# mauro3/KissMCMC.jl

Measured on AMD Instinct MI355X. Metric: walker-steps/sec, higher is better.
Workload: dtype f64

## Files before the change

### include/kissmcmc_hip.h

```cpp
#ifndef KISSMCMC_HIP_H
#define KISSMCMC_HIP_H

#include <stdint.h>

#ifdef __cplusplus
extern "C" {
#endif

#define KMC_VERSION 100

typedef enum kmc_status {
    KMC_OK = 0,
    KMC_ERR_A_SCALE = 1,
    KMC_ERR_ODD_WALKERS = 2,
    KMC_ERR_TOO_FEW_WALKERS = 3,
    KMC_ERR_BAD_ARG = 4,
    KMC_ERR_NONFINITE_LOGP = 5,
    KMC_ERR_HIP = 6,
    KMC_ERR_OOM = 7,
    KMC_ERR_NO_DEVICE = 8,
    KMC_ERR_UNSUPPORTED = 9
} kmc_status;

typedef enum kmc_density {
// ... 403 lines not shown
                                      int64_t* tail_len_j, int64_t* n_reff_nan, int64_t* n_out, int64_t* info);
kmc_status  kmc_chain_psis_loo_reff(kmc_user_density* density, const double* params, const double* chain_host, int64_t nsamples, int64_t nwalkers,
                                    int64_t ndim, int64_t first_sample, const uint8_t* walker_mask, int64_t thin, const double* r_eff_j,
                                    int32_t split, int64_t max_lag, int64_t obs_first, int64_t obs_count, int64_t workspace_bytes, int device,
                                    double* stats, double* lppd_j, double* r_eff_used, int64_t* tail_len_j, int64_t* n_reff_nan, int64_t* n_out,
                                    int64_t* info);
kmc_status  kmc_sampler_psis_tail_reff(kmc_sampler* s, int64_t first_sample, const uint8_t* walker_mask, int64_t thin, const double* r_eff_j,
                                       int32_t split, int64_t max_lag, int64_t obs_first, int64_t obs_count, int64_t workspace_bytes, double* tail,
                                       double* m_j, double* xc_j, int32_t* n_tail_j, int64_t* tail_len, double* r_eff_used, int64_t* tail_len_j,
                                       int64_t* n_reff_nan, int64_t* n_out);
kmc_status  kmc_chain_psis_tail_reff(kmc_user_density* density, const double* params, const double* chain_host, int64_t nsamples, int64_t nwalkers,
                                     int64_t ndim, int64_t first_sample, const uint8_t* walker_mask, int64_t thin, const double* r_eff_j,
                                     int32_t split, int64_t max_lag, int64_t obs_first, int64_t obs_count, int64_t workspace_bytes, int device,
                                     double* tail, double* m_j, double* xc_j, int32_t* n_tail_j, int64_t* tail_len, double* r_eff_used,
                                     int64_t* tail_len_j, int64_t* n_reff_nan, int64_t* n_out);

kmc_status  kmc_debug_accept_terms(uint64_t seed, uint64_t step, uint64_t walker0, int64_t n, int64_t nhalf, double a_scale,
                                   int64_t ndim, int device, int64_t* partner_host, double* z_host, double* t1_host, double* lu_host);
kmc_status  kmc_debug_chain_by_walker(const void* src_host, int is_float, int64_t K, int64_t nl, int64_t ld, int64_t nd, int64_t w0,
                                      int64_t nw, int64_t dst_stride, double* dst_host, int64_t dst_len, int device);
kmc_status  kmc_debug_rows_compact(const double* src_host, int64_t rows, int64_t ld, int64_t nd, double* dst_host, int64_t dst_len,
                                   int device);
int         kmc_debug_phase_spec(int density, int L, int K, int iter);

#ifdef __cplusplus
}
#endif
#endif
```

### kissmcmc.jl_amd/_lib.py

```python
from __future__ import annotations

import ctypes as C
import os

_HERE = os.path.dirname(os.path.abspath(__file__))
LIB_PATH = os.environ.get("KMC_LIB_PATH") or os.path.join(_HERE, "libkissmcmc_hip.so")

OK, ERR_A_SCALE, ERR_ODD_WALKERS, ERR_TOO_FEW_WALKERS, ERR_BAD_ARG, ERR_NONFINITE_LOGP, \
    ERR_HIP, ERR_OOM, ERR_NO_DEVICE, ERR_UNSUPPORTED = range(10)
GAUSSIAN_ISO, EXPONENTIAL, ROSENBROCK, LOGNORMAL, MVNORMAL2 = range(5)
USER_DENSITY = 100
HOST_DENSITY = 101
DATA_DENSITY = 102
HOST_LOGPDF_FN = C.CFUNCTYPE(C.c_int, C.POINTER(C.c_double), C.c_int64, C.c_int64, C.POINTER(C.c_double), C.c_void_p)
HOST_PROPOSE_FN = C.CFUNCTYPE(C.c_int, C.POINTER(C.c_double), C.c_int64, C.c_int64, C.POINTER(C.c_double), C.c_void_p)
HOST_ACCEPTED_FN = C.CFUNCTYPE(C.c_int, C.POINTER(C.c_uint8), C.c_int64, C.c_int64, C.c_int64, C.c_int32, C.c_void_p)
F64 = 0
F32 = 1
STORE_CHAIN, STORE_LOGP, MOMENTS, NO_GRAPH, P2P, ISLANDS, P2P_FINEGRAINED, P2P_PUSH = 1, 2, 4, 8, 16, 64, 128, 512
STREAM_CHAIN = 2048
CHAIN_BY_WALKER = 4096
STORE_BLOBS = 8192
MOVE_STRETCH, MOVE_DE, MOVE_SNOOKER, MOVE_MIX = 0, 1, 3, 4
MIX_MAX = 4
TEMPS_MAX = 64
CONV_NEED_LAGS, CONV_TRUNCATED = 1, 2
CONV_HAS_NAN = 4
TEMPER_WHOLE, TEMPER_LIKELIHOOD = 0, 1
P2P_HANDLE_BYTES = 128
RCCL_ID_BYTES = 128

SYMBOLS = [
    "kmc_version", "kmc_device_count", "kmc_last_error", "kmc_status_string", "kmc_validate",
    "kmc_g_pdf", "kmc_cdf_g_inv", "kmc_emcee_run", "kmc_sampler_create", "kmc_sampler_destroy",
    "kmc_sampler_set_stream", "kmc_sampler_bind_positions", "kmc_sampler_p2p_export", "kmc_sampler_p2p_connect", "kmc_sampler_p2p_connect_local", "kmc_sampler_p2p_link_probe", "kmc_sampler_set_positions", "kmc_sampler_init_ball", "kmc_sampler_set_state", "kmc_sampler_run", "kmc_sampler_half_step",
    "kmc_sampler_sync", "kmc_sampler_last_run_ms", "kmc_sampler_generation", "kmc_sampler_nsamples",
    "kmc_sampler_launch_count", "kmc_sampler_describe", "kmc_sampler_device_ptr", "kmc_sampler_get_positions",
    "kmc_sampler_get_logp", "kmc_sampler_get_naccept", "kmc_sampler_get_accept_ratio",
    "kmc_sampler_get_moments", "kmc_sampler_get_chain", "kmc_sampler_get_chain_by_walker", "kmc_logpdf_eval", "kmc_logpdf_eval_host",
    "kmc_user_density_create", "kmc_user_density_create_body", "kmc_user_density_destroy", "kmc_metropolis_validate", "kmc_metropolis_run", "kmc_cholesky_lower", "kmc_int_acorr", "kmc_sampler_int_acorr",
    "kmc_sizeof_config", "kmc_sizeof_metropolis_config", "kmc_sizeof_outputs", "kmc_sizeof_metropolis_outputs", "kmc_deal_seed", "kmc_deal_perm", "kmc_sampler_deal_pack", "kmc_sampler_deal_unpack",
    "kmc_sampler_get_walker_ids", "kmc_sampler_set_walker_ids", "kmc_sampler_set_chain_host", "kmc_rccl_unique_id", "kmc_sampler_rccl_init",
    "kmc_sampler_rccl_capture", "kmc_sampler_rccl_set_capture", "kmc_rccl_version", "kmc_device_free_bytes",
    "kmc_sampler_launch_mode", "kmc_updated_budget", "kmc_set_updated_budget_mb", "kmc_debug_accept_terms",
    "kmc_debug_chain_by_walker", "kmc_debug_rows_compact", "kmc_debug_phase_spec",
    "kmc_user_density_create_body_blob", "kmc_user_density_nblob", "kmc_logpdf_blob_eval_host", "kmc_sampler_get_blobs",
    "kmc_device_cache_release", "kmc_user_density_is_separable", "kmc_host_prefault", "kmc_data_density_create",
    "kmc_sampler_get_rung_state", "kmc_sampler_set_rung_state", "kmc_sampler_get_swaps",
    "kmc_sampler_get_rung_loglike", "kmc_sampler_set_rung_loglike_sum", "kmc_sampler_get_ladder", "kmc_sampler_set_ladder",
    "kmc_sampler_order_stats", "kmc_sampler_chain_argmax", "kmc_chain_order_stats", "kmc_chain_argmax",
    "kmc_sampler_histograms", "kmc_chain_histograms", "kmc_hist_pair_plan",
    "kmc_sampler_lag_sums", "kmc_chain_lag_sums", "kmc_convergence_stats", "kmc_sampler_convergence", "kmc_chain_convergence",
    "kmc_convergence_plan",
    "kmc_rank_plan", "kmc_rank_normal_scores", "kmc_sampler_rank_scores", "kmc_chain_rank_scores", "kmc_sampler_rank_convergence",
    "kmc_chain_rank_convergence",
    "kmc_sampler_hdi", "kmc_chain_hdi", "kmc_hdi_span",
    "kmc_sampler_covariance", "kmc_chain_covariance", "kmc_cov_plan", "kmc_cov_correlation",
    "kmc_sampler_pointwise_stats", "kmc_chain_pointwise_stats", "kmc_sampler_pointwise_loglike", "kmc_chain_pointwise_loglike",
    "kmc_pointwise_plan", "kmc_waic_stats",
    "kmc_sampler_psis_loo", "kmc_chain_psis_loo", "kmc_sampler_psis_tail", "kmc_chain_psis_tail", "kmc_psis_plan", "kmc_loo_stats",
    "kmc_psis_smooth_host",
    "kmc_sampler_relative_eff", "kmc_chain_relative_eff", "kmc_sampler_pointwise_weights", "kmc_chain_pointwise_weights",
    "kmc_sampler_psis_loo_reff", "kmc_chain_psis_loo_reff", "kmc_sampler_psis_tail_reff", "kmc_chain_psis_tail_reff",
]


class Config(C.Structure):
    _fields_ = [
# ... 265 lines not shown
    L.kmc_sampler_set_walker_ids.argtypes = [vp, ip]
    L.kmc_sampler_set_chain_host.argtypes = [vp, dp, dp]
    L.kmc_rccl_unique_id.argtypes = [vp]
    L.kmc_sampler_rccl_init.argtypes = [vp, vp]
    L.kmc_sampler_rccl_capture.argtypes = [vp, C.POINTER(C.c_int)]
    L.kmc_sampler_rccl_set_capture.argtypes = [vp, C.c_int]
    L.kmc_rccl_version.argtypes = [C.POINTER(C.c_int), C.c_char_p, C.c_int64]
    L.kmc_device_free_bytes.argtypes = [C.c_int, C.POINTER(C.c_uint64), C.POINTER(C.c_uint64)]
    L.kmc_device_cache_release.argtypes = []
    L.kmc_device_cache_release.restype = None
    L.kmc_host_prefault.argtypes = [C.c_void_p, C.c_uint64, C.c_int]
    L.kmc_host_prefault.restype = None
    L.kmc_sampler_launch_mode.restype = C.c_int
    L.kmc_sampler_launch_mode.argtypes = [vp, C.POINTER(C.c_int)]
    L.kmc_updated_budget.restype = None
    L.kmc_updated_budget.argtypes = [ip, ip]
    L.kmc_set_updated_budget_mb.restype = None
    L.kmc_set_updated_budget_mb.argtypes = [C.c_double]
    L.kmc_debug_accept_terms.argtypes = [C.c_uint64, C.c_uint64, C.c_uint64, C.c_int64, C.c_int64, C.c_double, C.c_int64, C.c_int, ip, dp, dp, dp]
    L.kmc_debug_chain_by_walker.argtypes = [vp, C.c_int, C.c_int64, C.c_int64, C.c_int64, C.c_int64, C.c_int64, C.c_int64, C.c_int64, dp, C.c_int64, C.c_int]
    L.kmc_debug_rows_compact.argtypes = [dp, C.c_int64, C.c_int64, C.c_int64, dp, C.c_int64, C.c_int]
    L.kmc_debug_phase_spec.restype = C.c_int
    L.kmc_debug_phase_spec.argtypes = [C.c_int, C.c_int, C.c_int, C.c_int]
    for fn, T in ((L.kmc_sizeof_config, Config), (L.kmc_sizeof_metropolis_config, MetropolisConfig),
                  (L.kmc_sizeof_outputs, Outputs), (L.kmc_sizeof_metropolis_outputs, MetropolisOutputs)):
        if fn() != C.sizeof(T):
            raise ImportError(f"{LIB_PATH}: struct layout mismatch ({fn.__name__}() = {fn()}, the ctypes mirror {T.__name__} is {C.sizeof(T)} bytes): "
                              "rebuild the library or update kissmcmc_jl_amd/_lib.py from include/kissmcmc_hip.h")
    _lib = L
    return L


def check(status: int) -> None:
    if status != OK:
        L = lib()
        msg = L.kmc_last_error().decode() or L.kmc_status_string(status).decode()
        raise KmcError(status, msg)
```

### kissmcmc.jl_amd/build.py

```python
from __future__ import annotations

import os
import shutil
import subprocess

_HERE = os.path.dirname(os.path.abspath(__file__))
CSRC = os.path.join(_HERE, "csrc")
LIB = os.path.join(_HERE, "libkissmcmc_hip.so")
SOURCES = ["kmc_sampler.hip", "kmc_plan.hip", "kmc_launch.hip", "kmc_updated.hip", "kmc_state.hip", "kmc_copy.hip", "kmc_rtc.hip", "kmc_p2p.hip", "kmc_metropolis_api.hip", "kmc_acorr.hip", "kmc_summary.hip", "kmc_hist.hip", "kmc_convergence.hip", "kmc_rank.hip", "kmc_hdi.hip", "kmc_cov.hip", "kmc_pointwise.hip", "kmc_rccl.hip", "kmc_diag.hip", "kmc_inst_host.hip", "kmc_inst_host_temper.hip", "kmc_inst_host_temper_snooker.hip", "kmc_data.hip"] + \
          [f"kmc_inst_{d}{part}.hip" for part in ("", "_var", "_p2p", "_lds", "_spec", "_de", "_snooker", "_temper", "_temper_snooker") for d in ("lognormal", "exponential", "gaussian_iso", "rosenbrock", "mvnormal2")]
HEADERS = ["kmc_psis_fit.hpp", "kmc_host.hpp", "kmc_sampler.hpp", "kmc_device.hpp", "kmc_kernels.hpp", "kmc_islands.hpp", "kmc_generation.hpp", "kmc_copy_kernels.hpp", "kmc_summary_kernels.hpp", "kmc_hist_kernels.hpp", "kmc_convergence_kernels.hpp", "kmc_convergence_host.hpp", "kmc_rank_kernels.hpp", "kmc_rank_host.hpp", "kmc_hdi_kernels.hpp", "kmc_cov_kernels.hpp", "kmc_chain_view.hpp", "kmc_chain_kernels.hpp", "kmc_metropolis.hpp", "kmc_tables.hpp", "kmc_recognise.hpp", "kmc_data.hpp", "kmc_pointwise.hpp", os.path.join("..", "..", "include", "kissmcmc_hip.h")]
PRELOAD = ["-mllvm", "-amdgpu-kernarg-preload-count=14"]
FLAGS = ["--offload-arch=gfx950", "-O3", "-std=c++17", "-fPIC", "-ffp-contract=off",
         "-fvisibility=hidden", "-Wall", "-Wno-unused-function"]


def _hipcc() -> str:
    for c in (shutil.which("hipcc"), "/opt/rocm/bin/hipcc"):
        if c and os.path.exists(c):
            return c
    raise RuntimeError("hipcc not found: the HIP library cannot be built")




def stale(lib: str = LIB) -> bool:
    if not os.path.exists(lib):
        return True
    t = os.path.getmtime(lib)
    deps = [os.path.join(CSRC, f) for f in SOURCES + HEADERS]
    return any(os.path.getmtime(d) > t for d in deps)


def build(force: bool = False, verbose: bool = False, extra_flags=(), out: str = LIB, preload: bool = True) -> str:
# ... 30 lines not shown
```

### kissmcmc.jl_amd/csrc/kmc_plan.hip

```cpp
#include <algorithm>
#include <cmath>
#include <cstdlib>
#include <cstring>

#include "kmc_sampler.hpp"

using namespace kmc;
using namespace kmc_host;

namespace kmc_host {
bool lookup(int density, int L, int K, int iter, bool p2p, bool ragged, bool f32, HalfStepFn* vec, HalfStepFn* gen)
{
    return with_density(density, false, [&](auto d) {
        using D = decltype(d);
        if (p2p && f32) { *vec = nullptr; *gen = nullptr; }
        else if (p2p) density_part<D, 2>(L, K, iter, ragged, false, vec, gen);
        else if (ragged || f32) density_part<D, 1>(L, K, iter, ragged, f32, vec, gen);
        else density_part<D, 0>(L, K, iter, false, false, vec, gen);
        return true;
    });
}

bool lookup_move(int move, int density, int L, int K, int iter, bool ragged, HalfStepFn* vec, HalfStepFn* gen)
{
    return with_density(density, false, [&](auto d) {
        if (move == KMC_MOVE_SNOOKER) density_part<decltype(d), 4>(L, K, iter, ragged, false, vec, gen);
        else if (move == KMC_MOVE_MIX) density_part<decltype(d), 5>(L, K, iter, ragged, false, vec, gen);
        else density_part<decltype(d), 3>(L, K, iter, ragged, false, vec, gen);
        return true;
    });
}

bool lookup_temper(int move, int density, int L, int K, int iter, bool ragged, HalfStepFn* vec, HalfStepFn* gen)
{
    return with_density(density, false, [&](auto d) {
        using D = decltype(d);
        if (move == KMC_MOVE_SNOOKER) temper_part<D, Move::Snooker>(L, K, iter, ragged, vec, gen);
        else if (move == KMC_MOVE_MIX) temper_part<D, Move::Mix>(L, K, iter, ragged, vec, gen);
        else if (move == KMC_MOVE_DE) temper_part<D, Move::DE>(L, K, iter, ragged, vec, gen);
        else temper_part<D, Move::Stretch>(L, K, iter, ragged, vec, gen);
        return true;
    });
}

HalfStepFn lookup_spec(int density, int L, int K, int iter)
{
    return with_density(density, HalfStepFn(nullptr), [&](auto d) { return spec_part<decltype(d)>(L, K, iter); });
}

LogpdfFn logpdf_fn(int density)
{
    return with_density(density, LogpdfFn(nullptr), [](auto d) { return logpdf_lookup<decltype(d)>(); });
}

bool resident_lane_wanted(int64_t ndim)
{
    std::string e;
    if (debug_opt("resident", &e) && e == "pair") return false;
    return ndim <= 8;
}
int lane_nd(int64_t ndim) { return (int)ndim; }

void philox_host(const uint32_t ctr[4], const uint32_t key[2], uint32_t out[4])
{
    uint32_t c0 = ctr[0], c1 = ctr[1], c2 = ctr[2], c3 = ctr[3], k0 = key[0], k1 = key[1];
    for (int r = 0; r < 10; ++r) {
        const uint64_t p0 = (uint64_t)0xD2511F53u * c0, p1 = (uint64_t)0xCD9E8D57u * c2;
        const uint32_t n0 = (uint32_t)(p1 >> 32) ^ c1 ^ k0, n2 = (uint32_t)(p0 >> 32) ^ c3 ^ k1;
        c0 = n0; c1 = (uint32_t)p1; c2 = n2; c3 = (uint32_t)p0;
        k0 += 0x9E3779B9u; k1 += 0xBB67AE85u;
// ... 72 lines not shown
            if (c.move == KMC_MOVE_SNOOKER) temper_part<HostEval, Move::Snooker>(1, 1, 1, false, &vec, &p.fn);
            else if (c.move == KMC_MOVE_MIX) temper_part<HostEval, Move::Mix>(1, 1, 1, false, &vec, &p.fn);
            else if (c.move == KMC_MOVE_DE) temper_part<HostEval, Move::DE>(1, 1, 1, false, &vec, &p.fn);
            else temper_part<HostEval, Move::Stretch>(1, 1, 1, false, &vec, &p.fn);
        }
        return p;
    }
    if (c.density == KMC_USER_DENSITY) {
        const kmc_user_density* ud = static_cast<const kmc_user_density*>(c.user_density);
        const bool body = ud && ud->is_body && !(sep_routed(ud) || body_vec_possible(ud, c.ndim));
        if (!body && !force_generic && L > 0 && 2 * L * K >= c.ndim && iter <= L && iter * K <= 16) {
            if (ud && ud->is_body && !sep_routed(ud)) while (iter > 1 && body_vec_lds_bytes(L, K, iter) > 65536) iter /= 2;
            p.vec = true; p.L = L; p.K = K; p.ITER = iter;
        } else {
            p.vec = false; p.L = 1; p.K = 1; p.ITER = 1;
        }
        return p;
    }
    if (tempered(c)) lookup_temper(c.move, c.density, L, K, iter, ragged, &vec, &gen);
    else if (de) lookup_move(c.move, c.density, L, K, iter, ragged, &vec, &gen);
    else lookup(c.density, L, K, iter, (c.flags & KMC_P2P) != 0, ragged, f32, &vec, &gen);
    if (!force_generic && L > 0 && 2 * L * K >= c.ndim && vec != nullptr) {
        p.fn = vec; p.vec = true; p.L = L; p.K = K; p.ITER = iter;
        if (!tempered(c) && !de && !(c.flags & KMC_P2P) && !ragged && !f32 && iter <= 2) p.fn_credit = lookup_spec(c.density, L, K, iter);
    } else {
        p.fn = gen; p.vec = false; p.L = 1; p.K = 1; p.ITER = 1;
    }
    return p;
}

kmc_status check_ndim(int density, int64_t ndim)
{
    if (density == KMC_ROSENBROCK && ndim < 2) return fail(KMC_ERR_BAD_ARG, "rosenbrock needs ndim >= 2");
    if (density == KMC_MVNORMAL2 && ndim != 2) return fail(KMC_ERR_BAD_ARG, "mvnormal2 needs ndim == 2");
    return KMC_OK;
}

}
kmc_status kmc_host::digest_params(const kmc_config& c, DensityParams* dp)
{
    for (double& v : dp->p) v = 0.0;
    dp->ndim = (int32_t)c.ndim;
    dp->pad_ = 0;
    const double* p = c.params;
    switch (c.density) {
    case KMC_USER_DENSITY:
        if (!c.user_density) return fail(KMC_ERR_BAD_ARG, "KMC_USER_DENSITY needs kmc_config.user_density");
// ... 13 lines not shown
        if (!(p[0] > 0.0)) return fail(KMC_ERR_BAD_ARG, "exponential: rate must be > 0");
        dp->p[0] = p[0];
        return KMC_OK;
    case KMC_ROSENBROCK:
        if (!(p[2] > 0.0)) return fail(KMC_ERR_BAD_ARG, "rosenbrock: scale must be > 0");
        dp->p[0] = p[0]; dp->p[1] = p[1]; dp->p[2] = 1.0 / p[2];
        return KMC_OK;
    case KMC_LOGNORMAL:
        if (!(p[1] > 0.0)) return fail(KMC_ERR_BAD_ARG, "lognormal: sigma must be > 0");
        dp->p[0] = p[0]; dp->p[1] = p[1];
        return KMC_OK;
    case KMC_MVNORMAL2:
        for (int i = 0; i < 5; ++i) dp->p[i] = p[i];
        return KMC_OK;
    default:
        return fail(KMC_ERR_BAD_ARG, "unknown density id");
    }
}

KMC_EXPORT int kmc_debug_phase_spec(int density, int L, int K, int iter)
{
    return kmc_host::lookup_spec(density, L, K, iter) != nullptr ? 1 : 0;
}
```

### kissmcmc.jl_amd/csrc/kmc_sampler.hip

```cpp
#include <algorithm>
#include <cmath>
#include <cstdio>
#include <cstdlib>
#include <mutex>
#include <random>
#include <sstream>

#include "kmc_sampler.hpp"

using namespace kmc;
using namespace kmc_host;

thread_local std::string kmc_host::g_err;

KMC_EXPORT int kmc_version(void) { return KMC_VERSION; }

KMC_EXPORT int kmc_device_count(void)
{
    int n = 0;
    if (hipGetDeviceCount(&n) != hipSuccess) { (void)hipGetLastError(); return 0; }
    return n;
}

KMC_EXPORT const char* kmc_last_error(void) { return g_err.c_str(); }
// ... 976 lines not shown
        else
            o << "one launch per generation (exact): generation_group L=" << s->fused_L << " K=" << s->plan.K << ", rows lane-striped, second-half walkers recompute their partner's first-half move, grid "
              << 2 * ((s->h + s->fused_tpb / s->fused_L - 1) / (s->fused_tpb / s->fused_L)) << " x " << s->fused_tpb;
        o << launch_mode_text(s, "generation");
    } else if (s->data_eval) {
        const DataPlan& ph = s->plan_half;
        const int64_t np = (int64_t)s->ntemps * s->h;
        o << "data density (exact): per half-step propose kernel -> " << (ph.obs ? "data_partial_obs (one observation per lane, grid " + std::to_string(np)
                                                                                 : "data_partial_lane (one proposal per lane, grid " + std::to_string((np + 63) / 64))
          << " x " << ph.nblocks << " workgroups of 256, " << ph.rounds << " rounds per wave) -> " << (s->temper_like ? "data_fold_split" : "data_fold") << " -> accept kernel, eager launches; "
          << s->data_ud->ndata << " observations of " << s->data_ud->ncols << " doubles; scratch " << ph.nblocks << " x " << np
          << " tree nodes (at most 4096 x " << (s->temper_like ? "ntemps x " : "") << "nwalkers doubles)";
    } else if (s->host_eval)
        o << "host-evaluated density (exact): per half-step propose kernel -> D2H -> callback -> H2D -> accept kernel, grid "
          << s->grid << " x 256";
    else if (s->plan.vec) {
        o << "multi-launch (exact): half_step_vec L=" << s->plan.L << " K=" << s->plan.K << " ITER=" << s->plan.ITER
          << (s->plan.ragged ? " ragged" : " exact-size") << ", grid " << s->grid << " x " << s->tpb
          << launch_mode_text(s, "step");
        if (s->launch_mode == 3 && !(s->cfg.flags & KMC_NO_GRAPH)) {
            const char* why = nullptr;
            if (spec_variant_possible(s, kVarCredit, &why)) o << "; phase-specialised kernel instance in counted replays";
            else o << "; generic kernel in every phase (" << why << ")";
        }
    } else
        o << "multi-launch (exact): " << (s->user && s->uk.staged ? "half_step_staged (one walker per lane, rows staged through LDS)" : "half_step_generic (one walker per lane)")
          << ", grid " << s->grid << " x " << s->tpb;
    if (s->feed_replays > 0 && debug_opt("feed-stats")) {
        char b[200];
        std::snprintf(b, sizeof(b), "; feeding thread per replay of %lld generations: wait for a free executable %.1f us, parameter updates %.1f us, hipGraphLaunch %.1f us (%lld replays)",
                      (long long)s->uchunk, s->feed_wait_ns / 1e3 / s->feed_replays, s->feed_update_ns / 1e3 / s->feed_replays, s->feed_launch_ns / 1e3 / s->feed_replays, (long long)s->feed_replays);
        o << b;
    }
    if (s->cfg.move == KMC_MOVE_DE) {
        char b[160];
        std::snprintf(b, sizeof(b), "; differential-evolution move (KMC_MOVE_DE): gamma0 %.6g, sigma %.3g, kernel %s", de_gamma0_of(s->cfg), s->cfg.de_sigma,
                      s->host_eval ? "half_step_de_generic (propose / accept passes)" : s->plan.vec ? "half_step_de_vec" : "half_step_de_generic");
        o << b;
    }
    if (s->cfg.move == KMC_MOVE_SNOOKER) {
        char b[160];
        std::snprintf(b, sizeof(b), "; snooker move (KMC_MOVE_SNOOKER): gamma %.6g, kernel %s", snooker_gamma_of(s->cfg.snooker_gamma),
                      s->host_eval ? "half_step_snooker_generic (propose / accept passes)" : s->plan.vec ? "half_step_snooker_vec" : "half_step_snooker_generic");
        o << b;
    }
    if (s->cfg.move == KMC_MOVE_MIX) {
// ... 59 lines not shown
            {"d_ring", s->d_ring}, {"d_draws", s->d_draws}, {"d_pos2", s->d_pos2}, {"d_glast", s->d_glast}, {"d_isum", s->d_isum}, {"d_msum", s->d_msum},
            {"d_mring", s->d_mring}, {"bw_scratch", s->bw_scratch}, {"bw_scratch_logp", s->bw_scratch_logp}, {"d_ids", s->d_ids}, {"d_mix", s->d_mix},
            {"d_like", s->d_like}, {"d_acc", s->d_acc}, {"d_prop", s->d_prop}, {"d_part", s->d_part}, {"d_betas", s->d_betas}, {"d_chain", s->d_chain},
            {"d_chain_logp", s->d_chain_logp}, {"d_blob", s->d_blob}, {"d_chain_blob", s->d_chain_blob}, {"d_err", s->d_err}};
        for (const auto& b : bufs) o << " " << b.first << "=" << (b.second != nullptr);
    }
    const std::string t = o.str();
    std::snprintf(buf, (size_t)buflen, "%s", t.c_str());
    return KMC_OK;
}

KMC_EXPORT void* kmc_sampler_device_ptr(kmc_sampler* s, int which)
{
    if (!s) return nullptr;
    if (which == 0 || which == 1) s->pos_exposed = true;
    switch (which) {
    case 0: return s->d_pos;
    case 1: return s->d_logp;
    case 2: return s->d_naccept;
    default: return nullptr;
    }
}


KMC_EXPORT int kmc_sizeof_config(void) { return (int)sizeof(kmc_config); }
KMC_EXPORT int kmc_sizeof_metropolis_config(void) { return (int)sizeof(kmc_metropolis_config); }
KMC_EXPORT int kmc_sizeof_outputs(void) { return (int)sizeof(kmc_outputs); }
KMC_EXPORT int kmc_sizeof_metropolis_outputs(void) { return (int)sizeof(kmc_metropolis_outputs); }
```

### kissmcmc.jl_amd/csrc/kmc_sampler.hpp

```cpp
#pragma once
#include <string>
#include <utility>
#include <vector>

#include "kmc_host.hpp"

KMC_EXPORT int kmc_version(void);

namespace kmc_host {

static_assert(1024 % kmc::kDrawBatch == 0, "the draw table holds whole batches");
constexpr int64_t kDrawTableGens = 1024;
constexpr int64_t kGraphChunk = 64;
constexpr int kUExec = 6;
enum : int { kVarGeneric = 0, kVarCredit = 1, kUVariants = 2 };
constexpr size_t kGuardBytes = 4096;
constexpr int kHostPieces = 8;

struct Plan {
    kmc::HalfStepFn fn = nullptr;
    kmc::HalfStepFn fn_credit = nullptr;
    bool vec = false;
    bool ragged = false;
    int L = 1, K = 1, ITER = 1;
};

struct UserKernels {
    hipModule_t mod = nullptr;
    std::shared_ptr<void> keep;
    hipFunction_t vec = nullptr, generic = nullptr, logpdf = nullptr, resident = nullptr, island = nullptr, init_ball = nullptr;
    hipFunction_t generation = nullptr;
    hipFunction_t staged = nullptr;
    hipFunction_t logpdf_sep = nullptr;
};

struct UserModuleSpec {
    enum class Resident { None, Pair, Lane, Lane2 };
    enum class Generation { None, Lane, Striped, Quad };
    bool vec = false;
    int L = 0, K = 0, iter = 0;
    bool ragged = false;
    Resident resident = Resident::None;
    int pair_K = 0;
    bool pair_ragged = false;
// ... 195 lines not shown
    return k < s->nsamples ? k : s->nsamples;
}

inline int64_t launches_per_generation(const kmc_sampler* s) { return s->fused ? 1 : 2; }

Plan make_plan(const kmc_config& c, int64_t n_active);
bool resident_lane_wanted(int64_t ndim);
int lane_nd(int64_t ndim);
void island_perm(uint64_t seed, int64_t epoch, int64_t N, int64_t* A, int64_t* C);
uint64_t deal_seed(uint64_t seed, int32_t rank);
void deal_perm(uint64_t seed, int64_t epoch, int32_t rank, int64_t S, int64_t* A, int64_t* C);

kmc_status ensure_graph(kmc_sampler* s);
kmc_status flush_moments_now(kmc_sampler* s);
kmc_status unfuse(kmc_sampler* s);
kmc::DrawConsts draw_consts(const kmc_sampler* s);
kmc::HalfStepArgs make_args(const kmc_sampler* s, int half, bool graph_mode, int64_t gen_offset);
kmc::HalfStepFront front_of(const kmc::HalfStepArgs& a, bool ragged_vec);
kmc::GenerationArgs make_generation_args(const kmc_sampler* s, int from, bool graph_mode, int64_t gen_offset);
kmc::GenerationFront generation_front_of(const kmc::GenerationArgs& a, int tpb);

bool updated_graph_possible(const kmc_sampler* s);
bool spec_variant_possible(const kmc_sampler* s, int variant, const char** why_not = nullptr);
int spec_of_chunk(const kmc_sampler* s, int64_t g0, int64_t n);
kmc_status ensure_updated_graph(kmc_sampler* s);
kmc_status launch_updated_graph(kmc_sampler* s, bool* launched);
void drop_updated_graph(kmc_sampler* s);
bool update_budget_left(const kmc_sampler* s);
void note_budget_spent(kmc_sampler* s);

hipError_t upload_rows(const kmc_sampler* s, double* dst_dev, const double* src_host, size_t rows);
hipError_t download_rows(const kmc_sampler* s, double* dst_host, const double* src_dev, size_t rows);
kmc_status chain_before(kmc_sampler* s, int64_t g_end);
kmc_status chain_after(kmc_sampler* s);
kmc_status chain_flush(kmc_sampler* s);
void chain_unregister(kmc_sampler* s);

kmc_status load_user(kmc_user_density* ud, const UserModuleSpec& spec, UserKernels* uk);
void set_offline_compiler_hint(bool wanted);
bool body_vec_possible(const kmc_user_density* ud, int64_t ndim);

kmc_status load_data(kmc_user_density* ud, int64_t ndim, DataKernels* dk);
std::string data_functor_source(const kmc_user_density* ud);
kmc_status data_on_device(kmc_user_density* ud, int dev, std::shared_ptr<void>* keep);
DataPlan data_plan(const kmc_user_density* ud, int64_t nprop);
hipError_t launch_data_eval(const DataKernels& dk, const kmc_user_density* ud, const DataPlan& p, const double* prop, int64_t nprop, int32_t ld,
// ... 9 lines not shown
```

### kissmcmc.jl_amd/csrc/kmc_tables.hpp

```cpp
#pragma once
#include <type_traits>
#include "kmc_islands.hpp"
#include "kmc_generation.hpp"
#include "kmc_metropolis.hpp"

namespace kmc {

using HalfStepFn = void (*)(KMC_FRONT_TYPES, const HalfStepArgs);
using LogpdfFn = void (*)(const LogpdfArgs);
using FlushFn = void (*)(const FlushArgs);
using IslandFn = void (*)(const IslandArgs);
using ResidentFn = void (*)(const ResidentArgs);
using GenerationFn = void (*)(KMC_GEN_FRONT_TYPES, const GenerationArgs);
using InitBallFn = void (*)(const InitBallArgs);
using MetropolisFn = void (*)(const MetropolisArgs);
using MetropolisTabledFn = void (*)(const MetropolisArgs, const double*, int);

template <class D, int PART> void density_part(int L, int K, int iter, bool ragged, bool f32, HalfStepFn* vec, HalfStepFn* gen);
template <class D, Move M> void temper_part(int L, int K, int iter, bool ragged, HalfStepFn* vec, HalfStepFn* gen);
template <class D> HalfStepFn spec_part(int L, int K, int iter);
template <class D> LogpdfFn logpdf_lookup();
template <class D> InitBallFn init_ball_lookup();
template <class D> IslandFn island_lookup(int S, int K, bool ragged);
template <class D> ResidentFn resident_lookup(int tpb, int K, bool ragged);
template <class D> ResidentFn resident_lane_lookup(int ndim, bool f32);
template <class D> ResidentFn resident_lane2_lookup(int ndim);
template <class D> GenerationFn generation_lane_lookup(int ndim);
template <class D> GenerationFn generation_group_lookup(int L, int K);
template <class D> MetropolisFn metropolis_lookup(int ndim);
template <class D> MetropolisTabledFn metropolis_tabled_lookup(int ndim);
template <class D> MetropolisFn metropolis_mv_lookup(int ndim);
HalfStepFn half_step_host();
HalfStepFn half_step_host_de();
HalfStepFn half_step_host_snooker();
HalfStepFn half_step_host_mix();

#ifdef KMC_TABLES_IMPL
template <class D, int L, int K, int ITER, bool P2P, bool RAGGED, class T, Move M>
HalfStepFn vec_one()
{
    if constexpr (ITER > L || ITER * K > 16 || ((M == Move::Snooker || M == Move::Mix) && ITER > 1 && ITER * K > 4)) return nullptr;
    else if constexpr (M == Move::Snooker) return half_step_snooker_vec<D, L, K, ITER, RAGGED>;
    else if constexpr (M == Move::Mix) return half_step_mix_vec<D, L, K, ITER, RAGGED>;
// ... 281 lines not shown
```

### kissmcmc.jl_amd/csrc/kmc_updated.hip

```cpp
#include <atomic>
#include <chrono>
#include <cstdio>

#include "kmc_sampler.hpp"

using namespace kmc;
using namespace kmc_host;

namespace kmc_host {

namespace {
struct ParamPack {
    HalfStepFront hf;
    HalfStepArgs ha;
    GenerationFront gf;
    GenerationArgs ga;
    void* ptrs[11];
    explicit ParamPack(bool fused)
    {
        if (fused) {
            ptrs[0] = &gf.sched; ptrs[1] = &gf.pin; ptrs[2] = &gf.lin; ptrs[3] = &gf.pout; ptrs[4] = &gf.seed_lo; ptrs[5] = &gf.seed_hi;
            ptrs[6] = &gf.h; ptrs[7] = &gf.nb; ptrs[8] = &gf.ld; ptrs[9] = &gf.gen; ptrs[10] = &ga;
        } else {
            ptrs[0] = &hf.pos; ptrs[1] = &hf.sched; ptrs[2] = &hf.ring_now; ptrs[3] = &hf.logp; ptrs[4] = &hf.gw0; ptrs[5] = &hf.nact_half;
            ptrs[6] = &hf.seed_lo; ptrs[7] = &hf.seed_hi; ptrs[8] = &hf.nhalf; ptrs[9] = &hf.step; ptrs[10] = &ha;
        }
    }
};

HalfStepFn variant_fn(const kmc_sampler* s, int variant)
{
    return variant == kVarCredit ? s->plan.fn_credit : s->plan.fn;
}

hipKernelNodeParams node_params(const kmc_sampler* s, int variant, ParamPack* pk)
{
    hipKernelNodeParams np{};
    if (s->fused) {
        np.func = s->user ? reinterpret_cast<void*>(s->uk.generation) : reinterpret_cast<void*>(s->generation_kernel);
        np.gridDim = dim3(2u * pk->ga.nb);
        np.blockDim = dim3((unsigned)s->fused_tpb);
        np.sharedMemBytes = 0u;
    } else {
        np.func = s->user ? reinterpret_cast<void*>(s->uk.vec) : reinterpret_cast<void*>(variant_fn(s, variant));
        np.gridDim = dim3((unsigned)s->grid);
        np.blockDim = dim3((unsigned)s->tpb);
        np.sharedMemBytes = s->user ? s->vec_lds : 0u;
    }
    np.kernelParams = pk->ptrs;
    np.extra = nullptr;
    return np;
}

template <class Visit>
kmc_status for_each_node(const kmc_sampler* s, int variant, int64_t g0, Visit&& visit)
{
    ParamPack pk(s->fused);
    const int64_t per_gen = launches_per_generation(s);
    for (int64_t k = 0; k < per_gen * s->uchunk; ++k) {
        const int64_t g = k / per_gen;
        if (s->fused) {
            pk.ga = make_generation_args(s, (int)(g & 1), false, g0 + g);
            pk.gf = generation_front_of(pk.ga, s->fused_tpb);
        } else {
            pk.ha = make_args(s, (int)(k & 1), false, g0 + g);
            pk.hf = front_of(pk.ha, s->ragged_vec());
        }
        KMC_TRY(visit(k, node_params(s, variant, &pk)));
    }
    return KMC_OK;
}
}

void drop_updated_graph(kmc_sampler* s)
{
    for (int i = 0; i < kUExec; ++i) {
        for (int v = 0; v < kUVariants; ++v)
            if (s->uexec[v][i]) { (void)hipGraphExecDestroy(s->uexec[v][i]); s->uexec[v][i] = nullptr; }
        if (s->udone[i]) { (void)hipEventDestroy(s->udone[i]); s->udone[i] = nullptr; }
        s->uinflight[i] = false;
    }
    s->unext = 0;
    for (int v = 0; v < kUVariants; ++v)
        if (s->ugraph[v]) { (void)hipGraphDestroy(s->ugraph[v]); s->ugraph[v] = nullptr; }
}

bool spec_variant_possible(const kmc_sampler* s, int variant, const char** why_not)
{
    const char* why = nullptr;
    std::string v;
    const int64_t per_wg = (int64_t)(s->tpb / 64) * (64 / s->plan.L) * s->plan.ITER;
    if (variant == kVarGeneric) return true;
    if (debug_opt("spec", &v) && v == "0") why = "KMC_DEBUG=spec=0";
    else if (s->user || s->fused || s->host_eval || !s->plan.vec) why = "not the two-launch vector route of a menu density";
    else if (variant_fn(s, variant) == nullptr) why = "no instance for this move, row type or geometry";
    else if (s->h_loc != (int64_t)s->grid * per_wg) why = "grid not full";
    else if (variant == kVarCredit && !s->d_msum) why = "moments off";
    else if (variant == kVarCredit && (s->d_chain || s->d_chain_logp || s->d_chain_blob)) why = "chain on";
    if (why_not) *why_not = why;
    return why == nullptr;
}

int spec_of_chunk(const kmc_sampler* s, int64_t g0, int64_t n)
{
    (void)n;
    if (g0 >= s->cfg.nburnin) return spec_variant_possible(s, kVarCredit) ? kVarCredit : kVarGeneric;
    return kVarGeneric;
}

bool updated_graph_possible(const kmc_sampler* s)
{
    if (s->p2p || s->host_eval || s->islands || s->resident || s->comm || s->updated_refused) return false;
    if (s->temper) return false;
    if (s->fused) return s->user ? s->uk.generation != nullptr : s->generation_kernel != nullptr;
    return s->user ? (s->plan.vec && s->uk.vec != nullptr) : s->plan.fn != nullptr;
}

kmc_status ensure_updated_graph(kmc_sampler* s)
{
    if (s->uexec[kVarGeneric][0]) return KMC_OK;
    for (int v = 0; v < kUVariants; ++v) {
        if (!spec_variant_possible(s, v)) continue;
        HIP_TRY(hipGraphCreate(&s->ugraph[v], 0));
        s->unodes[v].assign((size_t)(launches_per_generation(s) * s->uchunk), nullptr);
        hipGraphNode_t prev = nullptr;
        KMC_TRY(for_each_node(s, v, 0, [&](int64_t k, const hipKernelNodeParams& np) -> kmc_status {
            hipGraphNode_t node = nullptr;
            HIP_TRY(hipGraphAddKernelNode(&node, s->ugraph[v], prev ? &prev : nullptr, prev ? 1 : 0, &np));
            s->unodes[v][(size_t)k] = node;
// ... 89 lines not shown
```

Baseline: 8.973 billion.

## Add workgroup-shared draw kernel variant for burn-in replays

Adds a new half-step kernel variant for burn-in chunks in which one leader wave per two-wave workgroup computes the random draws (partner index, stretch z, log terms) and publishes them through LDS to its sibling wave. The aim is to cut the redundant RNG and log evaluations per walker and to overlap partner-row loads with the draw arithmetic. The variant is selected for graph chunks that lie entirely within burn-in, and it uses a different grid and block shape. In exchange it adds LDS barriers and more instances, and it only applies to L=8, K=2, ITER=2 geometry.

```diff
diff --git a/include/kissmcmc_hip.h b/include/kissmcmc_hip.h
--- a/include/kissmcmc_hip.h
+++ b/include/kissmcmc_hip.h
@@ -449,6 +449,8 @@
 kmc_status  kmc_debug_rows_compact(const double* src_host, int64_t rows, int64_t ld, int64_t nd, double* dst_host, int64_t dst_len,
                                    int device);
 int         kmc_debug_phase_spec(int density, int L, int K, int iter);
+int         kmc_debug_shared_draws(int density, int L, int K, int iter);
+int         kmc_debug_replay_variant(int density, int64_t nwalkers, int64_t ndim, int64_t nburnin, int64_t g0, int64_t n, int moments, int chain);
 
 #ifdef __cplusplus
 }
diff --git a/kissmcmc.jl_amd/_lib.py b/kissmcmc.jl_amd/_lib.py
--- a/kissmcmc.jl_amd/_lib.py
+++ b/kissmcmc.jl_amd/_lib.py
@@ -43,7 +43,7 @@
     "kmc_sampler_get_walker_ids", "kmc_sampler_set_walker_ids", "kmc_sampler_set_chain_host", "kmc_rccl_unique_id", "kmc_sampler_rccl_init",
     "kmc_sampler_rccl_capture", "kmc_sampler_rccl_set_capture", "kmc_rccl_version", "kmc_device_free_bytes",
     "kmc_sampler_launch_mode", "kmc_updated_budget", "kmc_set_updated_budget_mb", "kmc_debug_accept_terms",
-    "kmc_debug_chain_by_walker", "kmc_debug_rows_compact", "kmc_debug_phase_spec",
+    "kmc_debug_chain_by_walker", "kmc_debug_rows_compact", "kmc_debug_phase_spec", "kmc_debug_shared_draws", "kmc_debug_replay_variant",
     "kmc_user_density_create_body_blob", "kmc_user_density_nblob", "kmc_logpdf_blob_eval_host", "kmc_sampler_get_blobs",
     "kmc_device_cache_release", "kmc_user_density_is_separable", "kmc_host_prefault", "kmc_data_density_create",
     "kmc_sampler_get_rung_state", "kmc_sampler_set_rung_state", "kmc_sampler_get_swaps",
@@ -355,6 +355,10 @@
     L.kmc_debug_rows_compact.argtypes = [dp, C.c_int64, C.c_int64, C.c_int64, dp, C.c_int64, C.c_int]
     L.kmc_debug_phase_spec.restype = C.c_int
     L.kmc_debug_phase_spec.argtypes = [C.c_int, C.c_int, C.c_int, C.c_int]
+    L.kmc_debug_shared_draws.restype = C.c_int
+    L.kmc_debug_shared_draws.argtypes = [C.c_int, C.c_int, C.c_int, C.c_int]
+    L.kmc_debug_replay_variant.restype = C.c_int
+    L.kmc_debug_replay_variant.argtypes = [C.c_int, C.c_int64, C.c_int64, C.c_int64, C.c_int64, C.c_int64, C.c_int, C.c_int]
     for fn, T in ((L.kmc_sizeof_config, Config), (L.kmc_sizeof_metropolis_config, MetropolisConfig),
                   (L.kmc_sizeof_outputs, Outputs), (L.kmc_sizeof_metropolis_outputs, MetropolisOutputs)):
         if fn() != C.sizeof(T):
diff --git a/kissmcmc.jl_amd/build.py b/kissmcmc.jl_amd/build.py
--- a/kissmcmc.jl_amd/build.py
+++ b/kissmcmc.jl_amd/build.py
@@ -8,8 +8,9 @@
 CSRC = os.path.join(_HERE, "csrc")
 LIB = os.path.join(_HERE, "libkissmcmc_hip.so")
 SOURCES = ["kmc_sampler.hip", "kmc_plan.hip", "kmc_launch.hip", "kmc_updated.hip", "kmc_state.hip", "kmc_copy.hip", "kmc_rtc.hip", "kmc_p2p.hip", "kmc_metropolis_api.hip", "kmc_acorr.hip", "kmc_summary.hip", "kmc_hist.hip", "kmc_convergence.hip", "kmc_rank.hip", "kmc_hdi.hip", "kmc_cov.hip", "kmc_pointwise.hip", "kmc_rccl.hip", "kmc_diag.hip", "kmc_inst_host.hip", "kmc_inst_host_temper.hip", "kmc_inst_host_temper_snooker.hip", "kmc_data.hip"] + \
-          [f"kmc_inst_{d}{part}.hip" for part in ("", "_var", "_p2p", "_lds", "_spec", "_de", "_snooker", "_temper", "_temper_snooker") for d in ("lognormal", "exponential", "gaussian_iso", "rosenbrock", "mvnormal2")]
-HEADERS = ["kmc_psis_fit.hpp", "kmc_host.hpp", "kmc_sampler.hpp", "kmc_device.hpp", "kmc_kernels.hpp", "kmc_islands.hpp", "kmc_generation.hpp", "kmc_copy_kernels.hpp", "kmc_summary_kernels.hpp", "kmc_hist_kernels.hpp", "kmc_convergence_kernels.hpp", "kmc_convergence_host.hpp", "kmc_rank_kernels.hpp", "kmc_rank_host.hpp", "kmc_hdi_kernels.hpp", "kmc_cov_kernels.hpp", "kmc_chain_view.hpp", "kmc_chain_kernels.hpp", "kmc_metropolis.hpp", "kmc_tables.hpp", "kmc_recognise.hpp", "kmc_data.hpp", "kmc_pointwise.hpp", os.path.join("..", "..", "include", "kissmcmc_hip.h")]
+          [f"kmc_inst_{d}{part}.hip" for part in ("", "_var", "_p2p", "_lds", "_spec", "_share", "_de", "_snooker", "_temper", "_temper_snooker") for d in ("lognormal", "exponential", "gaussian_iso", "rosenbrock", "mvnormal2")
+           if (part, d) != ("_share", "mvnormal2")]
+HEADERS = ["kmc_psis_fit.hpp", "kmc_host.hpp", "kmc_sampler.hpp", "kmc_device.hpp", "kmc_kernels.hpp", "kmc_islands.hpp", "kmc_generation.hpp", "kmc_copy_kernels.hpp", "kmc_summary_kernels.hpp", "kmc_hist_kernels.hpp", "kmc_convergence_kernels.hpp", "kmc_convergence_host.hpp", "kmc_rank_kernels.hpp", "kmc_rank_host.hpp", "kmc_hdi_kernels.hpp", "kmc_cov_kernels.hpp", "kmc_chain_view.hpp", "kmc_chain_kernels.hpp", "kmc_metropolis.hpp", "kmc_tables.hpp", "kmc_shared_draws.hpp", "kmc_recognise.hpp", "kmc_data.hpp", "kmc_pointwise.hpp", os.path.join("..", "..", "include", "kissmcmc_hip.h")]
 PRELOAD = ["-mllvm", "-amdgpu-kernarg-preload-count=14"]
 FLAGS = ["--offload-arch=gfx950", "-O3", "-std=c++17", "-fPIC", "-ffp-contract=off",
          "-fvisibility=hidden", "-Wall", "-Wno-unused-function"]
diff --git a/kissmcmc.jl_amd/csrc/kmc_inst_exponential_share.hip b/kissmcmc.jl_amd/csrc/kmc_inst_exponential_share.hip
--- /dev/null
+++ b/kissmcmc.jl_amd/csrc/kmc_inst_exponential_share.hip
@@ -0,0 +1,6 @@
+#define KMC_TABLES_IMPL
+#include "kmc_shared_draws.hpp"
+
+namespace kmc {
+KMC_INSTANTIATE_SHARE(Exponential);
+}
diff --git a/kissmcmc.jl_amd/csrc/kmc_inst_gaussian_iso_share.hip b/kissmcmc.jl_amd/csrc/kmc_inst_gaussian_iso_share.hip
--- /dev/null
+++ b/kissmcmc.jl_amd/csrc/kmc_inst_gaussian_iso_share.hip
@@ -0,0 +1,13 @@
+#define KMC_TABLES_IMPL
+#include "kmc_shared_draws.hpp"
+
+namespace kmc {
+KMC_INSTANTIATE_SHARE(GaussianIso);
+}
+
+#ifdef KMC_PROBE
+extern "C" __attribute__((visibility("default"))) int kmc_probe_read_share(void* out)
+{
+    return (int)hipMemcpyFromSymbol(out, HIP_SYMBOL(kmc::g_probe), sizeof(kmc::g_probe));
+}
+#endif
diff --git a/kissmcmc.jl_amd/csrc/kmc_inst_lognormal_share.hip b/kissmcmc.jl_amd/csrc/kmc_inst_lognormal_share.hip
--- /dev/null
+++ b/kissmcmc.jl_amd/csrc/kmc_inst_lognormal_share.hip
@@ -0,0 +1,6 @@
+#define KMC_TABLES_IMPL
+#include "kmc_shared_draws.hpp"
+
+namespace kmc {
+KMC_INSTANTIATE_SHARE(LogNormal);
+}
diff --git a/kissmcmc.jl_amd/csrc/kmc_inst_rosenbrock_share.hip b/kissmcmc.jl_amd/csrc/kmc_inst_rosenbrock_share.hip
--- /dev/null
+++ b/kissmcmc.jl_amd/csrc/kmc_inst_rosenbrock_share.hip
@@ -0,0 +1,6 @@
+#define KMC_TABLES_IMPL
+#include "kmc_shared_draws.hpp"
+
+namespace kmc {
+KMC_INSTANTIATE_SHARE(Rosenbrock);
+}
diff --git a/kissmcmc.jl_amd/csrc/kmc_plan.hip b/kissmcmc.jl_amd/csrc/kmc_plan.hip
--- a/kissmcmc.jl_amd/csrc/kmc_plan.hip
+++ b/kissmcmc.jl_amd/csrc/kmc_plan.hip
@@ -46,6 +46,15 @@
 HalfStepFn lookup_spec(int density, int L, int K, int iter)
 {
     return with_density(density, HalfStepFn(nullptr), [&](auto d) { return spec_part<decltype(d)>(L, K, iter); });
+}
+
+HalfStepFn lookup_share(int density, int L, int K, int iter, int* share)
+{
+    *share = 0;
+    return with_density(density, HalfStepFn(nullptr), [&](auto d) -> HalfStepFn {
+        if constexpr (std::is_same<decltype(d), MvNormal2>::value) return nullptr;
+        else return share_part<decltype(d)>(L, K, iter, share);
+    });
 }
 
 LogpdfFn logpdf_fn(int density)
@@ -164,7 +173,10 @@
     else lookup(c.density, L, K, iter, (c.flags & KMC_P2P) != 0, ragged, f32, &vec, &gen);
     if (!force_generic && L > 0 && 2 * L * K >= c.ndim && vec != nullptr) {
         p.fn = vec; p.vec = true; p.L = L; p.K = K; p.ITER = iter;
-        if (!tempered(c) && !de && !(c.flags & KMC_P2P) && !ragged && !f32 && iter <= 2) p.fn_credit = lookup_spec(c.density, L, K, iter);
+        if (!tempered(c) && !de && !(c.flags & KMC_P2P) && !ragged && !f32 && iter <= 2) {
+            p.fn_credit = lookup_spec(c.density, L, K, iter);
+            p.fn_share_burnin = lookup_share(c.density, L, K, iter, &p.share_burnin);
+        }
     } else {
         p.fn = gen; p.vec = false; p.L = 1; p.K = 1; p.ITER = 1;
     }
@@ -224,3 +236,9 @@
 {
     return kmc_host::lookup_spec(density, L, K, iter) != nullptr ? 1 : 0;
 }
+
+KMC_EXPORT int kmc_debug_shared_draws(int density, int L, int K, int iter)
+{
+    int share = 0;
+    return kmc_host::lookup_share(density, L, K, iter, &share) != nullptr ? share : 0;
+}
diff --git a/kissmcmc.jl_amd/csrc/kmc_sampler.hip b/kissmcmc.jl_amd/csrc/kmc_sampler.hip
--- a/kissmcmc.jl_amd/csrc/kmc_sampler.hip
+++ b/kissmcmc.jl_amd/csrc/kmc_sampler.hip
@@ -1022,6 +1022,8 @@
             const char* why = nullptr;
             if (spec_variant_possible(s, kVarCredit, &why)) o << "; phase-specialised kernel instance in counted replays";
             else o << "; generic kernel in every phase (" << why << ")";
+            if (spec_variant_possible(s, kVarShareBurnin, &why)) o << "; workgroup-shared draws in burn-in replays (" << variant_share(s, kVarShareBurnin) << " waves per workgroup)";
+            else o << "; no workgroup-shared draws (" << why << ")";
         }
     } else
         o << "multi-launch (exact): " << (s->user && s->uk.staged ? "half_step_staged (one walker per lane, rows staged through LDS)" : "half_step_generic (one walker per lane)")
@@ -1127,6 +1129,18 @@
     }
 }
 
+KMC_EXPORT int kmc_debug_replay_variant(int density, int64_t nwalkers, int64_t ndim, int64_t nburnin, int64_t g0, int64_t n, int moments, int chain)
+{
+    static double some = 0.0;
+    kmc_sampler s;
+    s.cfg.density = density; s.cfg.nwalkers = nwalkers; s.cfg.ndim = ndim; s.cfg.nburnin = nburnin; s.cfg.shard_count = 1;
+    s.h = s.h_loc = nwalkers / 2;
+    s.plan = make_plan(s.cfg, s.h_loc);
+    setup_launch_geometry(&s);
+    s.d_msum = moments ? &some : nullptr;
+    s.d_chain = chain ? &some : nullptr;
+    return spec_of_chunk(&s, g0, n);
+}
 
 KMC_EXPORT int kmc_sizeof_config(void) { return (int)sizeof(kmc_config); }
 KMC_EXPORT int kmc_sizeof_metropolis_config(void) { return (int)sizeof(kmc_metropolis_config); }
diff --git a/kissmcmc.jl_amd/csrc/kmc_sampler.hpp b/kissmcmc.jl_amd/csrc/kmc_sampler.hpp
--- a/kissmcmc.jl_amd/csrc/kmc_sampler.hpp
+++ b/kissmcmc.jl_amd/csrc/kmc_sampler.hpp
@@ -13,13 +13,15 @@
 constexpr int64_t kDrawTableGens = 1024;
 constexpr int64_t kGraphChunk = 64;
 constexpr int kUExec = 6;
-enum : int { kVarGeneric = 0, kVarCredit = 1, kUVariants = 2 };
+enum : int { kVarGeneric = 0, kVarCredit = 1, kVarShareBurnin = 2, kUVariants = 3 };
 constexpr size_t kGuardBytes = 4096;
 constexpr int kHostPieces = 8;
 
 struct Plan {
     kmc::HalfStepFn fn = nullptr;
     kmc::HalfStepFn fn_credit = nullptr;
+    kmc::HalfStepFn fn_share_burnin = nullptr;
+    int share_burnin = 0;
     bool vec = false;
     bool ragged = false;
     int L = 1, K = 1, ITER = 1;
@@ -261,6 +263,7 @@
 
 bool updated_graph_possible(const kmc_sampler* s);
 bool spec_variant_possible(const kmc_sampler* s, int variant, const char** why_not = nullptr);
+int variant_share(const kmc_sampler* s, int variant);
 int spec_of_chunk(const kmc_sampler* s, int64_t g0, int64_t n);
 kmc_status ensure_updated_graph(kmc_sampler* s);
 kmc_status launch_updated_graph(kmc_sampler* s, bool* launched);
diff --git a/kissmcmc.jl_amd/csrc/kmc_shared_draws.hpp b/kissmcmc.jl_amd/csrc/kmc_shared_draws.hpp
--- /dev/null
+++ b/kissmcmc.jl_amd/csrc/kmc_shared_draws.hpp
@@ -0,0 +1,176 @@
+#pragma once
+#include "kmc_tables.hpp"
+
+namespace kmc {
+
+constexpr int kShareRound = 256;
+
+template <class Dens, int L, int K, int ITER, int SHARE>
+__device__ __forceinline__ void half_step_share_body(const HalfStepFront& f, const HalfStepArgs& a)
+{
+    static_assert(BlobTrait<Dens>::n == 0 && RowEvalTrait<Dens>::n == 0, "menu densities with a fragment form");
+    static_assert(ITER <= 2, "one or two walkers per group");
+    static_assert(SHARE == 2 && SHARE * ITER <= L, "two waves per workgroup (the leader rule below is written for two); the leader's lanes must cover every sibling's walkers");
+    constexpr int G = 64 / L;
+    constexpr int W = G * ITER;
+    constexpr int TPB = 64 * SHARE;
+    constexpr int64_t ld = 2 * L * K;
+    __shared__ uint32_t sh_partner[SHARE][W];
+    __shared__ double sh_z[SHARE][W], sh_t1[SHARE][W], sh_lu[SHARE][W];
+    double* const posT = f.pos;
+    const int tid   = blockIdx.x * TPB + threadIdx.x;
+    const int lane  = threadIdx.x & 63;
+    const int wv    = __builtin_amdgcn_readfirstlane((int)(threadIdx.x >> 6));
+    const int j     = lane & (L - 1);
+    const int g     = lane / L;
+    const int gbase = lane & ~(L - 1);
+    const int w0    = (tid >> 6) * W;
+    const int half  = f.half();
+    const int64_t own_row0 = (int64_t)f.gw0;
+    const int64_t oth_row0 = (int64_t)(1 - half) * (int64_t)f.nhalf;
+    const int lead = (int)(((unsigned)blockIdx.x / (2u * (unsigned)kShareRound)) & 1u);
+    KMC_STAMP(0);
+
+    const int  js   = j % ITER;
+    const bool useA = j < ITER;
+    const int  iA   = w0 + js * G + g;
+    const int64_t rowA = own_row0 + iA;
+
+    double2 xc[ITER][K], xo[ITER][K];
+#pragma unroll
+    for (int it = 0; it < ITER; ++it) {
+        const double2* own = reinterpret_cast<const double2*>(posT + (own_row0 + w0 + it * G + g) * ld);
+#pragma unroll
+        for (int k = 0; k < K; ++k) xc[it][k] = load_row(&own[k * L + j]);
+    }
+    const double p0 = f.logp[rowA];
+
+    const int  vL   = j / ITER;
+    const int  sL   = js * G + g;
+    const bool pubL = vL < SHARE;
+    const uint64_t step = (uint64_t)f.step;
+    DrawConsts dcf{};
+    dcf.seed_lo = f.seed_lo; dcf.seed_hi = f.seed_hi; dcf.nhalf = f.nhalf;
+    U4 bits{0u, 0u, 0u, 0u};
+    if (wv == lead) {
+        const int iL = ((int)blockIdx.x * SHARE + (pubL ? vL : SHARE - 1)) * W + sL;
+        bits = draw_bits(dcf, step, (uint64_t)f.gw0 + (uint64_t)iL);
+        if (pubL) sh_partner[vL][sL] = draw_partner(dcf, bits);
+    }
+    lds_barrier();
+    KMC_STAMP(1);
+
+    auto load_partner_rows = [&](int it) {
+        const uint32_t partner = sh_partner[wv][it * G + g];
+        const double2* oth = reinterpret_cast<const double2*>(posT + (oth_row0 + partner) * ld);
+#pragma unroll
+        for (int k = 0; k < K; ++k) xo[it][k] = load_row(&oth[k * L + j]);
+    };
+    constexpr int kFirst = ITER >= 2 ? ITER / 2 : ITER;
+#pragma unroll
+    for (int it = 0; it < kFirst; ++it) load_partner_rows(it);
+    __builtin_amdgcn_sched_barrier(0);
+    KMC_STAMP(2);
+
+    DrawConsts dc = a.dc;
+    dc.seed_lo = f.seed_lo; dc.seed_hi = f.seed_hi; dc.nhalf = f.nhalf;
+    KMC_STAMP(3);
+    double zL = 0.0, t1L = 0.0, luL = 0.0, ua = 0.5;
+    if (wv == lead) {
+        const double uz = ((double)bits.y + 0.5) * 0x1.0p-32;
+        const double t  = fma(uz, dc.c1, dc.c0);
+        zL = t * t;
+        const uint64_t kk = ((uint64_t)bits.z << 20) | (uint64_t)(bits.w >> 12);
+        ua = ((double)kk + 0.5) * 0x1.0p-52;
+        t1L = dc.nm1 * log_pos_normal(zL);
+    }
+    __builtin_amdgcn_sched_barrier(0);
+#pragma unroll
+    for (int it = kFirst; it < ITER; ++it) load_partner_rows(it);
+    __builtin_amdgcn_sched_barrier(0);
+    if (wv == lead) {
+        luL = log_pos_normal(ua);
+        if (pubL) { sh_z[vL][sL] = zL; sh_t1[vL][sL] = t1L; sh_lu[vL][sL] = luL; }
+    }
+    lds_barrier();
+    KMC_STAMP(4);
+    Draw dr;
+    dr.partner = 0u; dr.z = 0.0; dr.t1 = sh_t1[wv][js * G + g]; dr.lu = sh_lu[wv][js * G + g];
+    double zB[ITER];
+#pragma unroll
+    for (int it = 0; it < ITER; ++it) zB[it] = sh_z[wv][it * G + g];
+
+    double myp1 = 0.0;
+#pragma unroll
+    for (int it = 0; it < ITER; ++it) {
+#pragma unroll
+        for (int k = 0; k < K; ++k) {
+            xo[it][k].x = fma(zB[it], xc[it][k].x - xo[it][k].x, xo[it][k].x);
+            xo[it][k].y = fma(zB[it], xc[it][k].y - xo[it][k].y, xo[it][k].y);
+        }
+        if constexpr (MultiSumTrait<Dens>::n > 0) {
+            double S[MultiSumTrait<Dens>::n];
+            Dens::template frag_partial_n<L, K>(xo[it], j, 2 * L * K, a.dp, S);
+#pragma unroll
+            for (int q = 0; q < MultiSumTrait<Dens>::n; ++q) S[q] = group_sum<L>(S[q]);
+            const double p1 = Dens::finish_n(S, a.dp);
+            myp1 = (j == it) ? p1 : myp1;
+        } else {
+            const double S  = group_sum<L>(Dens::template frag_partial<L, K>(xo[it], j, 2 * L * K, a.dp));
+            const double p1 = Dens::finish(S, a.dp);
+            myp1 = (j == it) ? p1 : myp1;
+        }
+    }
+    KMC_STAMP(5);
+
+    const bool acc = useA && accept_test(dr, myp1, p0);
+    const unsigned long long accmask = __ballot(acc);
+    if (acc) store_wt(&f.logp[rowA], myp1);
+    KMC_STAMP(6);
+
+#pragma unroll
+    for (int it = 0; it < ITER; ++it) {
+        const bool accB = ((accmask >> (gbase + it)) & 1ull) != 0;
+        if (accB) {
+            double2* own = reinterpret_cast<double2*>(posT + (own_row0 + w0 + it * G + g) * ld);
+#pragma unroll
+            for (int k = 0; k < K; ++k) store_row(&own[k * L + j], xo[it][k]);
+        }
+    }
+    KMC_STAMP(7);
+#ifdef KMC_PROBE
+    {
+        unsigned long long st[8];
+        asm volatile("s_waitcnt lgkmcnt(0)" ::: "memory");
+        KMC_STAMP_READ(st[0], 80, 81); KMC_STAMP_READ(st[1], 82, 83); KMC_STAMP_READ(st[2], 84, 85); KMC_STAMP_READ(st[3], 86, 87);
+        KMC_STAMP_READ(st[4], 88, 89); KMC_STAMP_READ(st[5], 90, 91); KMC_STAMP_READ(st[6], 92, 93); KMC_STAMP_READ(st[7], 94, 95);
+        if (lane == 0 && (tid >> 6) < 8192) for (int q = 0; q < 8; q += (KMC_PROBE == 2 ? 7 : 1)) g_probe[half][tid >> 6][q] = st[q];
+    }
+#endif
+}
+
+template <class Dens, int L, int K, int ITER, int SHARE>
+__global__ __launch_bounds__(64 * SHARE) void half_step_vec_share(KMC_FRONT_PARAMS, const HalfStepArgs a)
+{
+    half_step_share_body<Dens, L, K, ITER, SHARE>(KMC_FRONT_PACK, a);
+}
+
+constexpr int kShareWaves = 2;
+
+#ifdef KMC_TABLES_IMPL
+template <class D>
+HalfStepFn share_part(int L, int K, int iter, int* share)
+{
+    *share = 0;
+    if constexpr (D::kHasFrag && BlobTrait<D>::n == 0 && RowEvalTrait<D>::n == 0) {
+        if (L == 8 && K == 2 && iter == 2) {
+            *share = kShareWaves;
+            return half_step_vec_share<D, 8, 2, 2, kShareWaves>;
+        }
+    }
+    return nullptr;
+}
+#define KMC_INSTANTIATE_SHARE(D) template HalfStepFn share_part<D>(int, int, int, int*)
+#endif
+
+}
diff --git a/kissmcmc.jl_amd/csrc/kmc_tables.hpp b/kissmcmc.jl_amd/csrc/kmc_tables.hpp
--- a/kissmcmc.jl_amd/csrc/kmc_tables.hpp
+++ b/kissmcmc.jl_amd/csrc/kmc_tables.hpp
@@ -19,6 +19,7 @@
 template <class D, int PART> void density_part(int L, int K, int iter, bool ragged, bool f32, HalfStepFn* vec, HalfStepFn* gen);
 template <class D, Move M> void temper_part(int L, int K, int iter, bool ragged, HalfStepFn* vec, HalfStepFn* gen);
 template <class D> HalfStepFn spec_part(int L, int K, int iter);
+template <class D> HalfStepFn share_part(int L, int K, int iter, int* share);
 template <class D> LogpdfFn logpdf_lookup();
 template <class D> InitBallFn init_ball_lookup();
 template <class D> IslandFn island_lookup(int S, int K, bool ragged);
diff --git a/kissmcmc.jl_amd/csrc/kmc_updated.hip b/kissmcmc.jl_amd/csrc/kmc_updated.hip
--- a/kissmcmc.jl_amd/csrc/kmc_updated.hip
+++ b/kissmcmc.jl_amd/csrc/kmc_updated.hip
@@ -30,7 +30,20 @@
 
 HalfStepFn variant_fn(const kmc_sampler* s, int variant)
 {
-    return variant == kVarCredit ? s->plan.fn_credit : s->plan.fn;
+    return variant == kVarCredit ? s->plan.fn_credit : variant == kVarShareBurnin ? s->plan.fn_share_burnin : s->plan.fn;
+}
+}
+
+int variant_share(const kmc_sampler* s, int variant)
+{
+    return variant == kVarShareBurnin ? s->plan.share_burnin : 0;
+}
+
+namespace {
+int64_t variant_walkers_per_wg(const kmc_sampler* s, int variant)
+{
+    const int share = variant_share(s, variant);
+    return (int64_t)(share > 0 ? share : s->tpb / 64) * (64 / s->plan.L) * s->plan.ITER;
 }
 
 hipKernelNodeParams node_params(const kmc_sampler* s, int variant, ParamPack* pk)
@@ -45,6 +58,10 @@
         np.func = s->user ? reinterpret_cast<void*>(s->uk.vec) : reinterpret_cast<void*>(variant_fn(s, variant));
         np.gridDim = dim3((unsigned)s->grid);
         np.blockDim = dim3((unsigned)s->tpb);
+        if (const int share = variant_share(s, variant); share > 0) {
+            np.gridDim = dim3((unsigned)(s->h_loc / variant_walkers_per_wg(s, variant)));
+            np.blockDim = dim3(64u * (unsigned)share);
+        }
         np.sharedMemBytes = s->user ? s->vec_lds : 0u;
     }
     np.kernelParams = pk->ptrs;
@@ -89,22 +106,23 @@
 {
     const char* why = nullptr;
     std::string v;
-    const int64_t per_wg = (int64_t)(s->tpb / 64) * (64 / s->plan.L) * s->plan.ITER;
+    const bool credits = variant == kVarCredit;
     if (variant == kVarGeneric) return true;
     if (debug_opt("spec", &v) && v == "0") why = "KMC_DEBUG=spec=0";
+    else if (variant == kVarShareBurnin && debug_opt("share", &v) && v == "0") why = "KMC_DEBUG=share=0";
     else if (s->user || s->fused || s->host_eval || !s->plan.vec) why = "not the two-launch vector route of a menu density";
     else if (variant_fn(s, variant) == nullptr) why = "no instance for this move, row type or geometry";
-    else if (s->h_loc != (int64_t)s->grid * per_wg) why = "grid not full";
-    else if (variant == kVarCredit && !s->d_msum) why = "moments off";
-    else if (variant == kVarCredit && (s->d_chain || s->d_chain_logp || s->d_chain_blob)) why = "chain on";
+    else if (s->h_loc != (int64_t)s->grid * variant_walkers_per_wg(s, kVarGeneric) || s->h_loc % variant_walkers_per_wg(s, variant) != 0) why = "grid not full";
+    else if (credits && !s->d_msum) why = "moments off";
+    else if (credits && (s->d_chain || s->d_chain_logp || s->d_chain_blob)) why = "chain on";
     if (why_not) *why_not = why;
     return why == nullptr;
 }
 
 int spec_of_chunk(const kmc_sampler* s, int64_t g0, int64_t n)
 {
-    (void)n;
     if (g0 >= s->cfg.nburnin) return spec_variant_possible(s, kVarCredit) ? kVarCredit : kVarGeneric;
+    if (g0 + n <= s->cfg.nburnin && spec_variant_possible(s, kVarShareBurnin)) return kVarShareBurnin;
     return kVarGeneric;
 }
 
```

Result: faster. 9.077 billion (median of 6 runs) (+1.1%).
